# nyashiki/nshogi-engine

Hardware: AMD Instinct MI355X
Metric: NN evals/sec at batch=512 (higher is better)
Workload: dtype f16m6 (f16 main term + e2m3 MX correction terms with per-32-channel E8M0 scales, f32 accumulate)

## Files before the change

### nshogi-engine_amd/csrc/kernels/mfma_tile.h

```cpp
#ifndef NSG_MFMA_TILE_H
#define NSG_MFMA_TILE_H

#include "kernels.h"

#include <atomic>
#include <type_traits>

namespace nsg {
namespace tile {

typedef float f32x4 __attribute__((ext_vector_type(4)));
typedef unsigned int u32x4 __attribute__((ext_vector_type(4)));
typedef unsigned int u32x2 __attribute__((ext_vector_type(2)));
typedef __bf16 bf16x8 __attribute__((ext_vector_type(8)));
typedef _Float16 f16x8 __attribute__((ext_vector_type(8)));

enum Mode { kConv = 0, kHeads = 1, kDense = 2 };

#ifdef NSG_COOP_SC1_STORES
constexpr bool kCoopSameXcd = false;
#else
constexpr bool kCoopSameXcd = true;
#endif
#ifdef NSG_COOP_NO_KEEP
constexpr bool kCoopKeepOwnSlice = false;
#else
constexpr bool kCoopKeepOwnSlice = true;
#endif
#ifdef NSG_NO_EDGE_ROWS_ONE_BOARD
constexpr bool kEdgeRowsOneBoard = false;
#else
constexpr bool kEdgeRowsOneBoard = true;
#endif

template <int MODE, int SIZE, int NWAVES, int NBUF = 2>
struct Geom {
    static constexpr bool kBoards = (MODE == kConv);
    static constexpr int kRows = kBoards ? SIZE * 81 : SIZE * 16;
    static constexpr int kMF = (kRows + 15) / 16;
    static constexpr int kEntries = kBoards ? SIZE * 110 + 24 : kMF * 16;
    static constexpr int kPlane = (kEntries * 16 + 7 * 16 + 255) / 256 * 256;
    static constexpr int kPlaneStride = kPlane + 16;
    static_assert(7 * kPlaneStride + kEntries * 16 <= 8 * kPlane, "the eight skewed planes must fit the buffer");
    static constexpr int kBuf = 8 * kPlane;
    static constexpr int kLds = NBUF * kBuf;
    static constexpr int kEpi = kLds;
    static constexpr int kRowTabOff = (kEpi > kLds ? kEpi : kLds) + 1024;
    static constexpr int kLdsAlloc = kRowTabOff + 1024;
    static constexpr int kThreads = NWAVES * 64;
    static constexpr int kItems = (2 * kMF + NWAVES - 1) / NWAVES;
    static constexpr int kTaps = kBoards ? 9 : 1;
};

template <bool BOARDS>
__device__ __forceinline__ int entryOfRow(int m) {
    if constexpr (BOARDS) {
        const int b = m / 81;
        const int sq = m - b * 81;
        const int y = sq / 9;
        const int x = sq - y * 9;
        return 24 + b * 110 + (y + 1) * 10 + x;
    } else {
        return m;
    }
}

template <class G, bool SHIFT = false>
__device__ __forceinline__ void zeroHalo(unsigned char* smem, int tid) {
    static_assert(G::kBoards, "board images only");
    constexpr int kBoardsN = (G::kEntries - 24) / 110;
    constexpr int kHalo = 24 + 29 * kBoardsN;
    constexpr int kPlanes = G::kLds / G::kPlane;
    const int lane = tid & 63, wave = tid >> 6;
    constexpr int kWavesN = G::kThreads / 64;
#pragma unroll
    for (int h0 = 0; h0 < kHalo; h0 += 64) {
        const int h = h0 + lane;
        int e = h;
        if (h0 + 63 >= 24) {
            const int q = h - 24, b = q / 29, r = q - b * 29;
            const int within = r < 10 ? r : (r < 19 ? (r - 9) * 10 + 9 : 81 + r);
            e = h < 24 ? h : 24 + b * 110 + within;
        }
        e = h < kHalo ? e : 0;
#pragma unroll
        for (int pl = 0; pl < (kPlanes + kWavesN - 1) / kWavesN; ++pl) {
            int plane = pl * kWavesN + wave;
            plane = plane < kPlanes ? plane : kPlanes - 1;
            if constexpr (SHIFT) {
                unsigned char* z = smem + e * 16 + (plane >> 3) * G::kBuf + (plane & 7) * G::kPlaneStride + ((plane & 7) == 7 ? 8 : 0);
                *reinterpret_cast<u32x2*>(z) = u32x2{0u, 0u};
                *reinterpret_cast<u32x2*>(z + 8) = u32x2{0u, 0u};
            } else {
                *reinterpret_cast<u32x4*>(smem + e * 16 + (plane >> 3) * G::kBuf + (plane & 7) * G::kPlaneStride) = u32x4{0u, 0u, 0u, 0u};
            }
        }
    }
}

template <int PREC>
__device__ __forceinline__ void mfmaSlab(f32x4& acc, const u32x4& w, const u32x4& a) {
    if constexpr (PREC == kFp32) {
        acc = __builtin_amdgcn_mfma_f32_16x16x4f32(__uint_as_float(w.x), __uint_as_float(a.x), acc, 0, 0, 0);
        acc = __builtin_amdgcn_mfma_f32_16x16x4f32(__uint_as_float(w.y), __uint_as_float(a.y), acc, 0, 0, 0);
        acc = __builtin_amdgcn_mfma_f32_16x16x4f32(__uint_as_float(w.z), __uint_as_float(a.z), acc, 0, 0, 0);
        acc = __builtin_amdgcn_mfma_f32_16x16x4f32(__uint_as_float(w.w), __uint_as_float(a.w), acc, 0, 0, 0);
    } else if constexpr (PREC == kFp16 || PREC == kF16x3) {
        acc = __builtin_amdgcn_mfma_f32_16x16x32_f16(__builtin_bit_cast(f16x8, w), __builtin_bit_cast(f16x8, a), acc, 0, 0, 0);
    } else {
        acc = __builtin_amdgcn_mfma_f32_16x16x32_bf16(__builtin_bit_cast(bf16x8, w), __builtin_bit_cast(bf16x8, a), acc, 0, 0, 0);
    }
}

template <int PREC>
__device__ __forceinline__ uint16_t toBits16(float v) {
    if constexpr (PREC == kFp16 || PREC == kF16x3) {
        return __builtin_bit_cast(uint16_t, (_Float16)v);
    } else {
        return __builtin_bit_cast(uint16_t, (__bf16)v);
    }
}
template <int PREC>
__device__ __forceinline__ uint32_t packPair(float lo, float hi) {
    return (uint32_t)toBits16<PREC>(lo) | ((uint32_t)toBits16<PREC>(hi) << 16);
}
template <int PREC>
__device__ __forceinline__ float unpackLo(uint32_t v) {
    if constexpr (PREC == kFp16) {
        return (float)__builtin_bit_cast(_Float16, (uint16_t)(v & 0xffffu));
    } else {
        return __uint_as_float(v << 16);
    }
}
__device__ __forceinline__ void splitF16(float v, uint16_t& hi, uint16_t& lo) {
    v = fminf(fmaxf(v, -65000.f), 65000.f);
    const _Float16 h = (_Float16)v;
    const _Float16 l = (_Float16)(v - (float)h);
    hi = __builtin_bit_cast(uint16_t, h);
    lo = __builtin_bit_cast(uint16_t, l);
}
// ... 203 lines not shown
    }
    static constexpr Tab kTab = make();
    static constexpr int kN = kTab.n, kMain = kTab.nMain, kX = kTab.nX;
    static constexpr int slab(int u) { return kTab.slab[u]; }
    static constexpr int mainOrd(int u) { return kTab.mainOrd[u]; }
    static constexpr int xOrd(int u) { return kTab.xOrd[u]; }
    static constexpr int mainSlab(int o) { return kTab.mainSlab[o]; }
    static constexpr int xSlab(int j) { return kTab.xSlab[j]; }
    static constexpr bool kXCyclic = kX >= 2 && kX % 2 == 0;
    static_assert(kMain % 3 == 0, "three f16 weight sets must carry across chunk pairs");
    static_assert(kX == 0 || kTab.xOrd[0] < 0 || kXCyclic, "a pair must not start with an MX slab it requests at its top");
};

template <class OS, int MF, bool PERM, int WIN, class ER>
struct StepSeq {
    static constexpr int kMax = (27 * MF + WIN - 1) / WIN * WIN;
    struct Tab {
        int n, padded;
        short pos[kMax], frag[kMax], index[27 * MF], xord[kMax];
    };
    static constexpr bool active(int u, int f) { return !PERM || ER::needTap(f, OS::slab(u) / 3); }
    static constexpr Tab make() {
        Tab t{};
        int n = 0;
        for (int u = 0; u < OS::kN; ++u)
            for (int f = 0; f < MF; ++f) {
                t.index[u * MF + f] = (short)(active(u, f) ? n : -1);
                if (active(u, f)) {
                    t.pos[n] = (short)u;
                    t.frag[n] = (short)f;
                    ++n;
                }
            }
        t.n = n;
        t.padded = (n + WIN - 1) / WIN * WIN;
        for (int q = n; q < kMax; ++q) { t.pos[q] = 0; t.frag[q] = -1; }
        int nx = 0;
        for (int q = 0; q < kMax; ++q) {
            t.xord[q] = (short)nx;
            if (q < n && OS::slab(t.pos[q]) % 3 == 2) ++nx;
        }
        return t;
    }
    static constexpr Tab kTab = make();
    static constexpr int kReal = kTab.n;
    static constexpr int kSteps = kTab.padded;
    static constexpr int pos(int q) { return kTab.pos[q]; }
    static constexpr int frag(int q) { return kTab.frag[q]; }
    static constexpr int index(int u, int f) { return kTab.index[u * MF + f]; }
    static constexpr int xord(int q) { return kTab.xord[q]; }
};

template <int PREC, int MODE, int SIZE, int NFRAG, int NWAVES, int RES, int MS = 1, int KS = 1, int SS = 1, int PART = 0, bool COOP = false,
          bool KEEP = false>
__device__ __forceinline__ void tileBody(const Args& A, unsigned char* smem, bool zeroLds, bool haveOwn = false) {
    static_assert(!KEEP || (COOP && SIZE == 1 && MS == 1 && KS > 1 && PREC == kF16m6), "own slice kept in LDS: cooperative K-split tiles");
    static_assert(!COOP || (isMx(PREC) && MODE == kConv && NFRAG == 4), "cooperative trunk: MX conv tiles");
    static_assert(SS == 1 || (isMx(PREC) && MODE == kConv && SIZE == 2 && MS == 1 && KS == 1 && NWAVES % SS == 0 && PART < SS),
                  "slab split: two-board MX conv tiles");
    using G = Geom<MODE, SIZE, NWAVES, (isMx(PREC) ? (KS > 1 ? 8 : 4) : 2)>;
    static_assert(KS == 1 || (isMx(PREC) && MODE == kConv && SIZE == 1 && NWAVES % KS == 0),
                  "K split: kF16m8 one-board conv tiles");
    constexpr bool kRowWG = (MS > 1 && KS > 1);
    const bool hasRes = (RES == 1) || (RES == 2 && A.res != nullptr);
    NSG_STAMP_DECL
    NSG_STAMP(0);
    constexpr bool kM8 = isMx(PREC);
    constexpr bool kM6 = (PREC == kF16m6);
    constexpr int ES = (PREC == kFp32 || PREC == kF16x3 || kM8) ? 4 : 2;
    constexpr bool kSplit = (PREC == kF16x3);
    static_assert(!kM8 || (MODE == kConv && NFRAG == 4), "kF16m8: full trunk-conv tiles only");
    static_assert(NFRAG == 1 || NFRAG == 2 || NFRAG == 4, "fragments per wave");
    static_assert(MS == 1 || (MODE == kConv && SIZE == 1 && G::kMF % MS == 0 && (KS > 1 || NWAVES % MS == 0) &&
                              (NFRAG < 4 || isMx(PREC))),
                  "row split: one-board conv tiles (small tiles, or kF16m8 full-channel tiles)");
    constexpr int kMFw = G::kMF / MS;
#ifdef NSG_NO_EDGE_ROWS
    constexpr bool kPerm = false;
#else
    constexpr bool kPerm = isMx(PREC) && MODE == kConv && NFRAG == 4 && MS == 1 && KS == 1 && (SIZE == 2 || (SIZE == 1 && kEdgeRowsOneBoard));
#endif
    using EdgeRows = std::conditional_t<SIZE == 1, EdgeRows1, EdgeRowsT<SS == 1>>;
    static_assert(!kPerm || kMFw == EdgeRows::kMF, "edge-packed rows: one table row per fragment");

    int tidOpaque = threadIdx.x;
    asm volatile("" : "+v"(tidOpaque));
    const int tid = tidOpaque;
    const int lane = tid & 63;
    const int wave = __builtin_amdgcn_readfirstlane(tid >> 6);
    const int li = lane & 15;
    const int g = lane >> 4;
    const size_t row0 = (size_t)blockIdx.x * G::kRows;
    int nkc = A.kdim * ES / 128;
    int kc0 = 0;
    if constexpr (MODE == kDense) {
        const int per = nkc / A.kSplits;
        kc0 = blockIdx.z * per;
        nkc = per;
    }
    const int nft = A.cout / 16;
    const int waveGroup = (blockIdx.y * NWAVES + wave) / (kRowWG ? KS : MS * KS * SS);
    const int fBase = (MS > 1) ? (kRowWG ? (int)blockIdx.z : wave % MS) * kMFw : 0;
    const int rowLimit = kRowWG ? ((fBase + kMFw) * 16 < G::kRows ? (fBase + kMFw) * 16 : G::kRows) : G::kRows;
    const size_t lastRow = G::kBoards ? ~(size_t)0 : (size_t)(A.totalRows - 1);

    const int sli = lane >> 3, sg = lane & 7;
    size_t srcOff[G::kItems];
    int dstOff[G::kItems];
    bool itemOk[G::kItems];
// ... 12 lines not shown
    if constexpr (kTileBuf) {
        xrs = __builtin_amdgcn_make_buffer_rsrc(const_cast<unsigned char*>(A.x) + row0 * (size_t)A.kdim * ES, 0, 0x7fffffff, 0x00027000);
#pragma unroll
        for (int k = 0; k < G::kItems; ++k) srcRel[k] = (int)(srcOff[k] - row0 * (size_t)A.kdim * ES);
    }
    auto tileLoad = [&](int k, int chunk) -> u32x4 {
        if constexpr (kTileBuf) return __builtin_bit_cast(u32x4, __builtin_amdgcn_raw_buffer_load_b128(xrs, srcRel[k], chunk * 128, COOP ? 16  : 0));
        else return *reinterpret_cast<const u32x4*>(A.x + srcOff[k] + (size_t)chunk * 128);
    };
    u32x4 st[G::kItems];
#ifdef NSG_MX_SPLIT_READ
    constexpr bool kShiftLo = (PREC == kF16m6) && MODE == kConv;
#else
    constexpr bool kShiftLo = false;
#endif
    auto stageStore = [](unsigned char* p_, const u32x4& v_) {
        if constexpr (kShiftLo) {
            *reinterpret_cast<u32x2*>(p_) = u32x2{v_.x, v_.y};
            *reinterpret_cast<u32x2*>(p_ + 8) = u32x2{v_.z, v_.w};
        } else {
            *reinterpret_cast<u32x4*>(p_) = v_;
        }
    };
    constexpr bool kResident = isMx(PREC) && KS > 1;
    constexpr int kResChunks = 8;
    constexpr int kOwnChunks = KEEP ? 2 * (NWAVES / KS) : 0;
    [[maybe_unused]] const int ownChunk0 = (int)blockIdx.y * kOwnChunks;
    u32x4 stAll[kResident ? kResChunks : 1][G::kItems];
    if constexpr (kResident) {
#pragma unroll
        for (int c = 0; c < kResChunks; ++c) {
            if (KEEP && haveOwn && c >= ownChunk0 && c < ownChunk0 + kOwnChunks) continue;
#pragma unroll
            for (int k = 0; k < G::kItems; ++k)
                stAll[c][k] = __builtin_bit_cast(u32x4, __builtin_amdgcn_raw_buffer_load_b128(
                    xrs, c < nkc ? srcRel[k] : 0x7ffffff0, c * 128, COOP ? 16  : 0));
        }
        __builtin_amdgcn_sched_barrier(0);
        NSG_STAMP(4);
    }
#pragma unroll
    for (int k = 0; k < G::kItems; ++k) {
        const int wid = wave + k * NWAVES;
        const int c = sg;
        const int mm = itemOk[k] ? wid * 8 + sli : 0;
        const int okOff = c * G::kPlaneStride + entryOfRow<G::kBoards>(mm) * 16 + ((kShiftLo && c == 7) ? 8 : 0), okMask = -(int)itemOk[k];
        dstOff[k] = (okOff & okMask) | ((G::kLds + lane * 16) & ~okMask);
    }

    int abase[kMFw];
    constexpr int kTabParts = KS > 1 ? KS : SS;
    constexpr int kTabFrags = (kMFw + kTabParts - 1) / kTabParts * kTabParts;
    static_assert(!kPerm || (kTabFrags + 1) * 64 <= 1024, "epilogue row table");
#define NSG_COMPUTE_ABASE \
_Pragma("unroll") \
    for (int f = 0; f < kMFw; ++f) { \
        [[maybe_unused]] int eb = 0, ey = 0, ex = 0; \
        [[maybe_unused]] bool eok = true; \
        if constexpr (kPerm) eok = EdgeRows::square(f, li, eb, ey, ex); \
        const int m = kPerm ? (eok ? eb * 81 + ey * 9 + ex : -1) : (fBase + f) * 16 + li; \
        if constexpr (kPerm) { \
            static_assert(NFRAG * 16 * ES == 256, "edge-packed rows: 256-byte row slices (4 rows per instruction)"); \
            if (wave == 0 && g == 0) { \
                reinterpret_cast<unsigned*>(smem + G::kRowTabOff)[(f * 4 + (li & 3)) * 4 + (li >> 2)] = \
                    m >= 0 ? (unsigned)m * (unsigned)(A.cout * ES) : ~0u; \
                 \
                if (f == kMFw - 1) { \
                    _Pragma("unroll") for (int fx = kMFw; fx <= kTabFrags; ++fx) \
                        reinterpret_cast<unsigned*>(smem + G::kRowTabOff)[(fx * 4 + (li & 3)) * 4 + (li >> 2)] = ~0u; \
                } \
            } \
        } \
        if constexpr (G::kBoards) { \
            const int p = kPerm ? (eok ? 24 + eb * 110 + (ey + 1) * 10 + ex : 11) \
                                : ((m < G::kRows) ? entryOfRow<true>(m) : 11); \
            abase[f] = g * G::kPlaneStride + (p - 11) * 16; \
        } else { \
            abase[f] = g * G::kPlaneStride + m * 16; \
        } \
    }
    if constexpr (!kPerm) { NSG_COMPUTE_ABASE }

#define NSG_PIN_ACC_AGPR                                                                 \
    _Pragma("unroll") for (int f = 0; f < kMFw; ++f) {                                   \
        _Pragma("unroll") for (int j = 0; j < NFRAG; ++j) asm volatile("" : "+a"(acc[f][j])); \
    }
#define NSG_STAGE_LOAD(KC)                                                               \
    _Pragma("unroll") for (int k = 0; k < G::kItems; ++k) {                              \
        st[k] = *reinterpret_cast<const u32x4*>(A.x + srcOff[k] + (size_t)(KC) * 128);   \
    }
#define NSG_STAGE_WRITE(BUF)                                                             \
    _Pragma("unroll") for (int k = 0; k < G::kItems; ++k) {                              \
        stageStore(smem + (itemOk[k] ? (BUF) * G::kBuf : 0) + dstOff[k], st[k]);         \
    }

    f32x4 acc[kMFw][NFRAG];
#pragma unroll
    for (int f = 0; f < kMFw; ++f)
#pragma unroll
        for (int j = 0; j < NFRAG; ++j) acc[f][j] = f32x4{0.f, 0.f, 0.f, 0.f};

    if constexpr (kM8) {
        using Q = M8Seq<G::kTaps>;
        using OS = OwnSeq<SS, PART>;
        static_assert(G::kTaps == 9, "3x3 taps");
        constexpr int kWin = 9, kD = 7;
#ifdef NSG_NO_SPREAD_LOADS
        constexpr bool kSpread = false;
#else
        constexpr bool kSpread = kMFw > NFRAG;
#endif
        using ST = StepSeq<OS, kMFw, kPerm, kWin, EdgeRows>;
        constexpr int kReal = ST::kReal;
        constexpr int kSteps = ST::kSteps;
        constexpr int kPad = kSteps - kReal;
        static_assert(kSteps % kWin == 0 && kPad < kD, "window slot must carry across chunk pairs");
        constexpr int kOwn = OS::kN;
        constexpr int kLoadSlabs = kOwn >= 20 ? (G::kItems < 6 ? G::kItems : 6) : (kOwn >= 12 ? 3 : 1);
        constexpr int kLoadSlabA = kOwn >= 20 ? 2 : 0, kWriteA = kOwn >= 20 ? 12 : (kOwn >= 12 ? 6 : 3);
        constexpr int kLoadSlabB = kOwn >= 20 ? 13 : kWriteA, kWriteB = kOwn >= 20 ? 25 : (kOwn >= 12 ? 12 : kOwn - 1);
        static_assert(kLoadSlabA + kLoadSlabs <= kWriteA && kLoadSlabB + kLoadSlabs <= kWriteB && kWriteB < kOwn, "tile staging order");
        constexpr int kBarStep = kReal - kD;
        constexpr int kWriteStepA = ST::index(kWriteA, 0), kWriteStepB = ST::index(kWriteB, 0) < kBarStep ? ST::index(kWriteB, 0) : kBarStep - 1;
        static_assert(kWriteStepA >= 0 && ST::index(kWriteB, 0) >= 0 && kWriteStepA < kWriteStepB, "fragment 0 runs every tap");
        static_assert(kWriteStepB < kBarStep, "tile staging order");
        auto tapOff = [](int t) constexpr { return ((t / 3 - 1) * 10 + (t % 3 - 1) + 11) * 16; };
        const int offp8 = (g >> 1) * G::kBuf + (4 + 2 * (g & 1) - g) * G::kPlaneStride;
        constexpr bool kPackX = kM6;
        const int mainSet = nft * 1024, xSet = nft * (kPackX ? 1600 : 2048);
        const int tapStride = 2 * mainSet + xSet, pairStride = G::kTaps * tapStride;
        int tapS = tapStride, mainS = mainSet;
        auto mainOff = [&](int s) { return (s / 3) * tapS + (s % 3) * mainS; };
        auto xOff = [&](int s) { return (s / 3) * tapS + 2 * mainS; };
        constexpr bool kStage = (KS == 1);
        const int kpart = (KS > 1) ? wave % KS : 0;
        const int npairs = nkc / 2 / KS;
        const int pair0 = kpart * npairs;
        const __amdgpu_buffer_rsrc_t wrs = __builtin_amdgcn_make_buffer_rsrc(const_cast<u32x4*>(A.w), 0, 0x7fffffff, 0x00027000);
        int wc = pair0 * pairStride;
        const int wg4 = waveGroup * NFRAG * 1024;
        const int wg8 = kPackX ? waveGroup * 6400 : waveGroup * NFRAG * 2048;
        const int lane16 = lane * 16, lane8 = lane * 8, lane4 = lane * 4;
        auto ld16 = [&](int off_, int imm_) { return __builtin_bit_cast(u32x4, __builtin_amdgcn_raw_buffer_load_b128(wrs, lane16 + imm_, off_, 0)); };
        auto ld8 = [&](int off_, int imm_) { return __builtin_bit_cast(u32x2, __builtin_amdgcn_raw_buffer_load_b64(wrs, lane8 + imm_, off_, 0)); };
        auto ld4 = [&](int off_, int imm_) { return (uint32_t)__builtin_amdgcn_raw_buffer_load_b32(wrs, lane4 + imm_, off_, 0); };
        u32x4 w4[OS::kMain > 0 ? 3 : 1][NFRAG];
        u32x4 w8[OS::kX > 0 ? 2 : 1][NFRAG][kPackX ? 1 : 2];
        [[maybe_unused]] u32x2 w8b[OS::kX > 0 ? 2 : 1][NFRAG];
        [[maybe_unused]] uint32_t w8s[OS::kX > 0 ? 2 : 1];
#define NSG_M8_LOADX(SET_, OFF_, J_)                                                                            \
        _Pragma("unroll") for (int j_ = 0; j_ < NFRAG; ++j_) {                                                  \
            if ((J_) >= 0 && j_ != (J_)) continue;                                                              \
            if constexpr (kPackX) {                                                                             \
                w8[SET_][j_][0] = ld16(wc + (OFF_) + wg8, j_ * 1024);                                           \
                w8b[SET_][j_] = ld8(wc + (OFF_) + wg8 + 4096, j_ * 512);                                        \
                if ((J_) < 0 ? j_ == 0 : (J_) == 0) w8s[SET_] = ld4(wc + (OFF_) + wg8 + 4096, 2048);            \
            } else {                                                                                            \
                _Pragma("unroll") for (int h_ = 0; h_ < 2; ++h_)                                                \
                    w8[SET_][j_][kPackX ? 0 : h_] = ld16(wc + (OFF_) + wg8 + (j_ >> 1) * 4096, ((j_ & 1) * 2 + h_) * 1024); \
            }                                                                                                   \
        }
        if constexpr (OS::kMain > 0) {
#pragma unroll
            for (int o = 0; o < 2; ++o)
#pragma unroll
                for (int j = 0; j < NFRAG; ++j) w4[o][j] = ld16(wc + mainOff(OS::mainSlab(o)) + wg4, j * 1024);
        }
        if constexpr (OS::kXCyclic) { NSG_M8_LOADX(0, xOff(OS::xSlab(0)), -1) }

        if constexpr (kStage) {
        u32x4 st1[G::kItems];
#pragma unroll
        for (int k = 0; k < G::kItems; ++k) st[k] = tileLoad(k, 0);
#pragma unroll
        for (int k = 0; k < G::kItems; ++k) st1[k] = tileLoad(k, 1);
        NSG_STAMP(4);
        if constexpr (kPerm) { NSG_COMPUTE_ABASE }
        if (zeroLds) zeroHalo<G, kShiftLo>(smem, tid);
        __syncthreads();
        NSG_STAMP(5);
        NSG_STAGE_WRITE(0)
#pragma unroll
        for (int k = 0; k < G::kItems; ++k)
            stageStore(smem + (itemOk[k] ? G::kBuf : 0) + dstOff[k], st1[k]);
        __syncthreads();
        } else {
            constexpr int kChunks = kResChunks;
            if constexpr (kPerm) { NSG_COMPUTE_ABASE }
            if (zeroLds) zeroHalo<G, kShiftLo>(smem, tid);
            __syncthreads();
            NSG_STAMP(5);
#pragma unroll
            for (int c = 0; c < kChunks; ++c) {
                if (KEEP && haveOwn && c >= ownChunk0 && c < ownChunk0 + kOwnChunks) continue;
#pragma unroll
                for (int k = 0; k < G::kItems; ++k)
                    if (__builtin_expect(c < nkc, 1)) stageStore(smem + (itemOk[k] ? c * G::kBuf : 0) + dstOff[k], stAll[c][k]);
            }
            __syncthreads();
        }
        NSG_STAMP(1);

        constexpr bool kSplitRead = kShiftLo && OS::kX > 0;
        const int offB = offp8 + G::kPlaneStride + 8 * (g & 1);
        u32x4 aw[kWin][kSplitRead ? 1 : 2];
        [[maybe_unused]] u32x2 aw45[kSplitRead ? kWin : 1];
        [[maybe_unused]] uint32_t awS[kSplitRead ? kWin : 1];
#define NSG_M8_REQ(QQ, CUR, NXT)                                                                  \
        if (ST::frag((QQ) % kSteps) >= 0) {                                                       \
            const int q_ = (QQ) % kSteps;                                                         \
            const unsigned char* b_ = ((QQ) >= kSteps) ? (NXT) : (CUR);                           \
            const int s_ = OS::slab(ST::pos(q_)), f_ = ST::frag(q_);                              \
            if (Q::isX(s_)) {                                                                     \
                const unsigned char* ap_ = b_ + abase[f_] + offp8 + tapOff(Q::tap(s_));           \
                aw[(QQ) % kWin][0] = *reinterpret_cast<const u32x4*>(ap_);                        \
                [[maybe_unused]] const unsigned char* ap2_ = b_ + abase[f_] + offB + tapOff(Q::tap(s_)); \
                if constexpr (kSplitRead) {                                                       \
                    aw45[(QQ) % kWin] = *reinterpret_cast<const u32x2*>(ap2_);                    \
                    awS[(QQ) % kWin] = *reinterpret_cast<const uint32_t*>(ap2_ + 12);             \
                } else if constexpr (kShiftLo) {                                                  \
                    aw[(QQ) % kWin][kSplitRead ? 0 : 1] = *reinterpret_cast<const u32x4*>(ap2_);  \
                } else {                                                                          \
                    aw[(QQ) % kWin][kSplitRead ? 0 : 1] = *reinterpret_cast<const u32x4*>(ap_ + G::kPlaneStride); \
                }                                                                                 \
            } else {                                                                              \
                aw[(QQ) % kWin][0] = *reinterpret_cast<const u32x4*>(                             \
                    b_ + Q::half(s_) * G::kBuf + abase[f_] + tapOff(Q::tap(s_)));                 \
            }                                                                                     \
        }
        const unsigned char* first = kStage ? smem : smem + (size_t)(2 * pair0) * G::kBuf;
#pragma unroll
        for (int q = 0; q < kD - kPad; ++q) NSG_M8_REQ(q, first, first)

        for (int kp = 0; kp < npairs; ++kp) {
            const unsigned char* abuf = kStage ? smem + ((2 * kp) & 3) * G::kBuf : smem + (size_t)(2 * (pair0 + kp)) * G::kBuf;
            const unsigned char* nbuf = kStage ? smem + ((2 * kp + 2) & 3) * G::kBuf
                                               : (kp + 1 < npairs ? abuf + 2 * G::kBuf : abuf);
            [[maybe_unused]] const int nextA = (kp + 1 < npairs) ? 2 * kp + 2 : 2 * kp;
// ... 387 lines not shown
                            const f32x4 rr = *reinterpret_cast<const f32x4*>(A.res + e + j * 16);
#pragma unroll
                            for (int i = 0; i < 4; ++i) v[j * 4 + i] += rr[i];
                        } else {
                            const u32x2 rr = *reinterpret_cast<const u32x2*>(A.res + e + j * 8);
                            v[j * 4 + 0] += unpackLo<PREC>(rr.x); v[j * 4 + 1] += unpackHi<PREC>(rr.x);
                            v[j * 4 + 2] += unpackLo<PREC>(rr.y); v[j * 4 + 3] += unpackHi<PREC>(rr.y);
                        }
                    }
                }
                if (A.relu) {
#pragma unroll
                    for (int i = 0; i < NFRAG * 4; ++i) v[i] = reluF(v[i]);
                }
#pragma unroll
                for (int j = 0; j < NFRAG; ++j) {
                    if constexpr (PREC == kFp32) {
                        *reinterpret_cast<f32x4*>(A.y + e + j * 16) = f32x4{v[j * 4], v[j * 4 + 1], v[j * 4 + 2], v[j * 4 + 3]};
                    } else {
                        *reinterpret_cast<u32x2*>(A.y + e + j * 8) =
                            u32x2{packPair<PREC>(v[j * 4], v[j * 4 + 1]), packPair<PREC>(v[j * 4 + 2], v[j * 4 + 3])};
                    }
                }
            }
        }
        NSG_STAMP(3);
        return;
    }

#ifdef NSG_EXP_RUNTIME
    if constexpr (MODE == kConv && NFRAG == 4 && isMx(PREC)) {
        if (A.exp & 2) {
#pragma unroll
            for (int f = 0; f < kMFw; ++f)
#pragma unroll
                for (int j = 0; j < NFRAG; ++j) asm volatile("" ::"v"(acc[f][j]));
            NSG_STAMP(3);
            return;
        }
    }
#endif
    if constexpr (MODE == kConv && NFRAG == 4) {
        constexpr int kParts = KS > 1 ? KS : SS;
        constexpr int kMFe = (kMFw + kParts - 1) / kParts;
        const int fBaseE = fBase + ((KS > 1) ? (wave % KS) * kMFe : PART * kMFe);
        constexpr int kRowB = NFRAG * 16 * ES;
        constexpr int kRowS = kRowB + 16;
        constexpr int kNP = kRowB / 64;
        constexpr int kPPR = kRowB / 16;
        constexpr int kRPI = 64 / kPPR;
        constexpr int kIPF = 16 / kRPI;
        constexpr int kFragBytes = 16 * kRowS;
        constexpr int kEpiWave = G::kEpi / NWAVES / 16 * 16;
        constexpr int kRegions = (kEpiWave / kFragBytes) < 1 ? 1 : ((kEpiWave / kFragBytes) > 4 ? 4 : (kEpiWave / kFragBytes));
        static_assert(kFragBytes <= kEpiWave, "epilogue staging does not fit");
        unsigned char* ebuf = smem + wave * kEpiWave;
        const size_t rowBytes = (size_t)A.cout * ES;
        const size_t sliceOff = (size_t)waveGroup * kRowB;
        auto pieceOff = [&](int k) -> int {
            if constexpr (kSplit || kM6) return (g >> 1) * 128 + (g & 1) * 32 + (k & 1) * 16 + (k >> 1) * 64;
            else if constexpr (kM8)
                return (g >> 1) * 128 + (k < 2 ? (g & 1) * 32 + k * 16 : 64 + (k - 2) * 32 + (g & 1) * 16);
            else return g * (kRowB / 4) + k * 16;
        };
        const bool outX3 = kM8 && A.outF16x3;
        auto pieceOffX3 = [&](int k) -> int { return (g >> 1) * 128 + (g & 1) * 32 + (k & 1) * 16 + (k >> 1) * 64; };
        const int lrow = lane / kPPR;
        const int lpc = lane % kPPR;
        const unsigned laneOff = (unsigned)lrow * (unsigned)rowBytes + (unsigned)lpc * 16u;
        const size_t tileOff = (row0 + (kPerm ? (size_t)0 : (size_t)fBaseE * 16)) * rowBytes + sliceOff;
        const unsigned char* resBase = A.res + tileOff;
        unsigned char* yBase = A.y + tileOff;
        [[maybe_unused]] __amdgpu_buffer_rsrc_t resRs, yRs;
        if constexpr (COOP) {
            resRs = __builtin_amdgcn_make_buffer_rsrc(const_cast<unsigned char*>(resBase), 0, 0x7fffffff, 0x00027000);
            yRs = __builtin_amdgcn_make_buffer_rsrc(yBase, 0, 0x7fffffff, 0x00027000);
        }
        auto resLoad = [&](size_t off_) -> u32x4 {
            if constexpr (COOP) return __builtin_bit_cast(u32x4, __builtin_amdgcn_raw_buffer_load_b128(resRs, (int)off_, 0, 16));
            else return *reinterpret_cast<const u32x4*>(resBase + off_);
        };
        auto outStore = [&](size_t off_, const u32x4& v_) {
            if constexpr (COOP) __builtin_amdgcn_raw_buffer_store_b128(v_, yRs, (int)off_, 0, kCoopSameXcd ? 0 : 16);
            else *reinterpret_cast<u32x4*>(yBase + off_) = v_;
        };
        [[maybe_unused]] const unsigned permLane = (unsigned)lpc * 16u;
        const int fBasePerm = (KS > 1) ? (wave % KS) * kMFe : PART * kMFe;
        auto rowOffs = [&](int f) -> u32x4 {
            if constexpr (kPerm) return *reinterpret_cast<const u32x4*>(smem + G::kRowTabOff + ((fBasePerm + f) * 4 + lrow) * 16);
            else return u32x4{0u, 0u, 0u, 0u};
        };
        auto rowOk = [&](int f, int it, const u32x4& ro) -> bool {
            if constexpr (kPerm) return (SIZE == 2 && KS == 1 && PART * kMFe + f < EdgeRows::kMF - 1) || ro[it] != ~0u;
            else return (fBaseE + f) * 16 + it * kRPI + lrow < rowLimit;
        };
        auto rowByte = [&](int f, int it, const u32x4& ro) -> size_t {
            if constexpr (kPerm) return (size_t)(ro[it] + permLane);
            else return (size_t)(f * 16 + it * kRPI) * rowBytes + laneOff;
        };

        constexpr int kPreFrags = (RES != 1 || minWavesPerSimd<MODE, SIZE, NWAVES, NFRAG, PREC>() > 1)
                                      ? 0 : (kMFe * kIPF <= 32 ? kMFe : 32 / kIPF);
        u32x4 rpre[kPreFrags ? kPreFrags : 1][kIPF];
        if constexpr (kPreFrags > 0) {
#pragma unroll
            for (int f = 0; f < kPreFrags; ++f) {
                const u32x4 ro = rowOffs(f);
#pragma unroll
                for (int it = 0; it < kIPF; ++it) {
                    rpre[f][it] = u32x4{0u, 0u, 0u, 0u};
                    if (__builtin_expect(rowOk(f, it, ro), 1))
                        rpre[f][it] = resLoad(rowByte(f, it, ro));
                }
            }
        }

        static_assert(kRegions >= 2, "the pipelined epilogue needs two staging regions per wave");
        [[maybe_unused]] int entLi[KEEP ? kMFe : 1], entLL[KEEP ? kMFe : 1][kIPF];
        if constexpr (KEEP) {
            static_assert(kRowB == 256 && kIPF == 4, "image staging: 256-byte row slices");
            const int slice_ = waveGroup * 2 * G::kBuf;
            auto entryByte = [&](int m_) { return m_ < G::kRows ? slice_ + (34 + m_ + ((m_ * 57) >> 9)) * 16 : -1; };
            auto rowOfFrag = [&](int fg_, int r_) -> int {
                if constexpr (kPerm) {
                    int b_ = 0, y_ = 0, x_ = 0;
                    const bool ok_ = EdgeRows::square(fg_ < EdgeRows::kMF ? fg_ : 0, r_, b_, y_, x_) && fg_ < EdgeRows::kMF;
                    return ok_ ? y_ * 9 + x_ : G::kRows;
                } else {
                    return fg_ * 16 + r_;
                }
            };
#pragma unroll
            for (int f = 0; f < kMFe; ++f) {
                entLi[f] = entryByte(rowOfFrag(fBaseE + f, li));
#pragma unroll
                for (int it = 0; it < kIPF; ++it) entLL[f][it] = entryByte(rowOfFrag(fBaseE + f, it * kRPI + lrow));
            }
        }
        auto stageAt = [&](int f, int rowIsLi, int it, int piece_) -> unsigned char* {
            if constexpr (KEEP) {
                const int e_ = rowIsLi ? entLi[f] : entLL[f][it];
                return smem + (e_ < 0 ? G::kLds + lane * 16 : e_ + (piece_ >> 3) * G::kBuf + (piece_ & 7) * G::kPlaneStride);
            } else {
                return ebuf + (f % kRegions) * kFragBytes + (rowIsLi ? li : it * kRPI + lrow) * kRowS + piece_ * 16;
            }
        };
        u32x4 rpp[2][kNP];
        u32x4 tt[kIPF];
#pragma unroll
        for (int i = -1; i <= kMFe; ++i) {
            [[maybe_unused]] u32x4 roS = u32x4{0u, 0u, 0u, 0u}, roR = u32x4{0u, 0u, 0u, 0u};
            if (i >= 1) {
                const int f = i - 1;
#pragma unroll
                for (int it = 0; it < kIPF; ++it)
                    tt[it] = *reinterpret_cast<const u32x4*>(stageAt(f, 0, it, lpc));
                roS = rowOffs(f);
            }
            if (hasRes && i + 1 < kMFe) {
                const int f = i + 1;
                if (f >= kPreFrags) roR = rowOffs(f);
                const u32x4 ro = roR;
#pragma unroll
                for (int it = 0; it < kIPF; ++it) {
                    u32x4 t = u32x4{0u, 0u, 0u, 0u};
                    if (f < kPreFrags) {
                        t = rpre[f < kPreFrags ? f : 0][it];
                    } else {
                        if (__builtin_expect(rowOk(f, it, ro), 1))
                            t = resLoad(rowByte(f, it, ro));
                    }
                    *reinterpret_cast<u32x4*>(stageAt(f, 0, it, lpc)) = t;
                }
#pragma unroll
                for (int k = 0; k < kNP; ++k) {
                    const int po = (kM6 && k >= 2) ? (g >> 1) * 128 + 96 + (k - 2) * 16 : pieceOff(k);
                    rpp[f & 1][k] = *reinterpret_cast<const u32x4*>(stageAt(f, 1, 0, po / 16));
                }
            }
            if (i >= 0 && i < kMFe) {
                const int f = i;
                float v[NFRAG * 4];
#pragma unroll
                for (int j = 0; j < NFRAG; ++j)
#pragma unroll
                    for (int r = 0; r < 4; ++r) v[j * 4 + r] = fmaf(acc[f][j][r], A.accScale, bv[j * 4 + r]);
                [[maybe_unused]] unsigned char* lrowp = ebuf + (f % kRegions) * kFragBytes + li * kRowS;
                if (hasRes) {
                    const u32x4* rp = rpp[f & 1];
                    if constexpr (PREC == kFp32) {
#pragma unroll
                        for (int k = 0; k < 4; ++k)
#pragma unroll
                            for (int i = 0; i < 4; ++i) v[k * 4 + i] += __uint_as_float(rp[k][i]);
                    } else if constexpr (kSplit) {
#pragma unroll
                        for (int k = 0; k < 2; ++k)
#pragma unroll
                            for (int i = 0; i < 4; ++i) {
// ... 110 lines not shown
                            sb[d] = sw.y;
                        }
                        const uint32_t mbits = __builtin_bit_cast(uint32_t, __builtin_convertvector(f32x2{mh, ml}, f16x2));
                        const uint32_t mhb = mbits & 0xffffu, mlb = mbits >> 16;
                        op[0] = u32x4{hpv[0], hpv[1], hpv[2], hpv[3]};
                        op[1] = u32x4{hpv[4], hpv[5], hpv[6], hpv[7]};
                        const u32x16 src = {sa[0], sa[1], sa[2], sa[3], sa[4], sa[5], sa[6], sa[7],
                                            sb[0], sb[1], sb[2], sb[3], sb[4], sb[5], sb[6], sb[7]};
                        const u32x2v mm = __builtin_amdgcn_permlane16_swap(mhb, mlb, false, false);
                        const uint32_t e5 = (mm.x > mm.y ? mm.x : mm.y) >> 10;
                        const uint32_t e8 = e5 + 110u;
                        u32x6 blk;
                        const float sc = __uint_as_float(e8 << 23);
                        asm("v_cvt_scalef32_pk32_fp6_f16 %0, %1, %2" : "=&v"(blk) : "v"(src), "v"(sc));
                        op[2] = u32x4{blk.s0, blk.s1, blk.s2, blk.s3};
                        op[3] = u32x4{blk.s4, blk.s5, e8, e8};
                    } else {
                        typedef float f32x2 __attribute__((ext_vector_type(2)));
                        typedef _Float16 f16x2 __attribute__((ext_vector_type(2)));
#pragma unroll
                        for (int d = 0; d < 4; ++d) {
                            f32x2 hf[2], lf[2];
#pragma unroll
                            for (int q = 0; q < 2; ++q) {
                                const int c = 4 * d + 2 * q;
                                const f32x2 x = {__builtin_amdgcn_fmed3f(v[c], floorV, 65000.f),
                                                 __builtin_amdgcn_fmed3f(v[c + 1], floorV, 65000.f)};
                                const f16x2 h = __builtin_convertvector(x, f16x2);
                                op[c >> 3][(c & 7) >> 1] = __builtin_bit_cast(uint32_t, h);
                                const f32x2 hx = __builtin_convertvector(h, f32x2);
                                const f32x2 lx = (x - hx) * (float)(1 << kM8LoShift);
                                hf[q] = f32x2{__builtin_amdgcn_fmed3f(hx[0], -448.f, 448.f), __builtin_amdgcn_fmed3f(hx[1], -448.f, 448.f)};
                                lf[q] = f32x2{__builtin_amdgcn_fmed3f(lx[0], -448.f, 448.f), __builtin_amdgcn_fmed3f(lx[1], -448.f, 448.f)};
                            }
                            int h8 = __builtin_amdgcn_cvt_pk_fp8_f32(hf[0][0], hf[0][1], 0, false);
                            h8 = __builtin_amdgcn_cvt_pk_fp8_f32(hf[1][0], hf[1][1], h8, true);
                            int l8 = __builtin_amdgcn_cvt_pk_fp8_f32(lf[0][0], lf[0][1], 0, false);
                            l8 = __builtin_amdgcn_cvt_pk_fp8_f32(lf[1][0], lf[1][1], l8, true);
                            op[2][d] = (uint32_t)h8;
                            op[3][d] = (uint32_t)l8;
                        }
                    }
                } else {
#pragma unroll
                    for (int k = 0; k < 2; ++k)
#pragma unroll
                        for (int i = 0; i < 4; ++i) op[k][i] = packPair<PREC>(v[k * 8 + 2 * i], v[k * 8 + 2 * i + 1]);
                }
#pragma unroll
                for (int k = 0; k < kNP; ++k) {
                    if constexpr (KEEP) *reinterpret_cast<u32x4*>(stageAt(f, 1, 0, (__builtin_expect(outX3, false) ? pieceOffX3(k) : pieceOff(k)) / 16)) = op[k];
                    else *reinterpret_cast<u32x4*>(lrowp + (__builtin_expect(outX3, false) ? pieceOffX3(k) : pieceOff(k))) = op[k];
                }
            }
            if (i >= 1) {
                const int f = i - 1;
                const u32x4 ro = roS;
#pragma unroll
                for (int it = 0; it < kIPF; ++it) {
#ifdef NSG_EXP_RUNTIME
                    asm volatile("" ::"v"(tt[it]));
                    if (__builtin_expect(rowOk(f, it, ro) && !(A.exp & 1), 1))
#else
                    if (__builtin_expect(rowOk(f, it, ro), 1))
#endif
                        outStore(rowByte(f, it, ro), tt[it]);
                }
            }
        }
#ifdef NSG_DIAG_STAMPS
        asm volatile("s_waitcnt vmcnt(0)" ::: "memory");
#endif
        NSG_STAMP(3);
        return;
    }

#pragma unroll
    for (int f = 0; f < G::kMF; ++f) {
        const int m = f * 16 + li;
        const size_t grow = row0 + m;
        const bool rowOk = G::kBoards ? (m < G::kRows) : (grow <= lastRow);
        if (!rowOk) continue;
        float v[NFRAG * 4];
#pragma unroll
        for (int j = 0; j < NFRAG; ++j)
#pragma unroll
            for (int r = 0; r < 4; ++r) v[j * 4 + r] = fmaf(acc[f][j][r], A.accScale, bv[j * 4 + r]);

        if constexpr (MODE == kHeads) {
            const int b = (int)(grow / 81);
            const int sq = (int)(grow - (size_t)b * 81);
            const int vc = A.valueChannels;
#pragma unroll
            for (int i = 0; i < NFRAG * 4; ++i) {
                const int n = cbase + i;
                if (n < vc) {
                    const float r = reluF(v[i]);
                    const size_t e = (size_t)b * A.vfeatStride + (size_t)sq * vc + n;
                    if constexpr (kSplit) {
                        const int kk = sq * vc + n;
                        uint16_t hb, lb;
                        splitF16(r, hb, lb);
                        unsigned char* row = A.vfeat + (size_t)b * A.vfeatStride * 4 + (size_t)(kk >> 5) * 128 + (kk & 31) * 2;
                        *reinterpret_cast<uint16_t*>(row) = hb;
                        *reinterpret_cast<uint16_t*>(row + 64) = lb;
                    } else if constexpr (PREC == kFp32) {
                        reinterpret_cast<float*>(A.vfeat)[e] = r;
                    } else {
                        reinterpret_cast<uint16_t*>(A.vfeat)[e] = toBits16<PREC>(r);
                    }
                } else if (n < vc + 27) {
                    A.policy[(size_t)b * 2187 + (size_t)(n - vc) * 81 + sq] = v[i];
                }
            }
        } else {
            float* out = reinterpret_cast<float*>(A.y) + (size_t)blockIdx.z * A.partStride + grow * (size_t)A.cout + cbase;
#pragma unroll
            for (int j = 0; j < NFRAG; ++j)
                *reinterpret_cast<f32x4*>(out + j * 4) =
                    f32x4{acc[f][j][0] * A.accScale, acc[f][j][1] * A.accScale, acc[f][j][2] * A.accScale, acc[f][j][3] * A.accScale};
        }
    }
}

template <int PREC, int MODE, int SIZE, int NFRAG, int NWAVES, bool HAS_RES, int MS = 1, int KS = 1, int SS = 1>
__global__ __launch_bounds__(NWAVES * 64, (minWavesPerSimd<MODE, SIZE, NWAVES, NFRAG, PREC>())) void tileKernel(
    const unsigned char* x, const u32x4* w, const unsigned char* res, unsigned char* y, const float* bias,
    int kdim, int cout, int flags , float accScale, const ArgsTail T) {
    extern __shared__ __attribute__((aligned(16))) unsigned char smem[];
    const Args A{x, w, bias, res, y, T.policy, T.vfeat, kdim, cout, T.totalRows, flags & 1, T.valueChannels,
                 T.vfeatStride, accScale, (flags >> 1) & 1, T.kSplits, T.partStride, T.stamps, flags >> 2};
    if constexpr (SS == 1) {
        tileBody<PREC, MODE, SIZE, NFRAG, NWAVES, HAS_RES ? 1 : 0, MS, KS>(A, smem, true);
    } else {
        const int part = __builtin_amdgcn_readfirstlane((int)(threadIdx.x >> 6)) % SS;
        if (part == 0) tileBody<PREC, MODE, SIZE, NFRAG, NWAVES, HAS_RES ? 1 : 0, MS, KS, SS, 0>(A, smem, true);
        else if (part == 1) tileBody<PREC, MODE, SIZE, NFRAG, NWAVES, HAS_RES ? 1 : 0, MS, KS, SS, 1>(A, smem, true);
        else if constexpr (SS > 2) {
            if (part == 2) tileBody<PREC, MODE, SIZE, NFRAG, NWAVES, HAS_RES ? 1 : 0, MS, KS, SS, 2>(A, smem, true);
            else tileBody<PREC, MODE, SIZE, NFRAG, NWAVES, HAS_RES ? 1 : 0, MS, KS, SS, 3>(A, smem, true);
        }
    }
}

template <int PREC, int SIZE, int NFRAG, int NWAVES>
__global__ __launch_bounds__(NWAVES * 64, (minWavesPerSimd<kConv, SIZE, NWAVES, NFRAG, PREC>())) void trunkKernel(
    const Args* __restrict__ layers, int nLayers, int skewTicks) {
    extern __shared__ __attribute__((aligned(16))) unsigned char smem[];
    if (skewTicks > 0) {
        const unsigned long long t0 = __builtin_amdgcn_s_memrealtime();
        const unsigned long long wait = (unsigned long long)skewTicks * ((blockIdx.x >> 3) & 7);
        while (__builtin_amdgcn_s_memrealtime() - t0 < wait) __builtin_amdgcn_s_sleep(16);
    }
    for (int l = 0; l < nLayers; ++l) {
        const Args A = layers[l];
        if (A.res) tileBody<PREC, kConv, SIZE, NFRAG, NWAVES, 1>(A, smem, true);
        else tileBody<PREC, kConv, SIZE, NFRAG, NWAVES, 0>(A, smem, true);
        __syncthreads();
    }
}

template <int PREC, int NFRAG, int NWAVES, int MS, int KS>
__global__ __launch_bounds__(NWAVES * 64, 1) void coopTrunkKernel(const Args* __restrict__ layers, int nLayers, int boards,
                                                                  unsigned* flags, unsigned flagBase, int* status, int faultBoard) {
    extern __shared__ __attribute__((aligned(16))) unsigned char smem[];
    using G = Geom<kConv, 1, NWAVES, 8>;
    if ((int)blockIdx.x >= boards) return;
    const int members = (int)(gridDim.y * gridDim.z), me = (int)(blockIdx.z * gridDim.y + blockIdx.y);
    if ((int)blockIdx.x == faultBoard && me == 1) return;
    unsigned xcc = 0;
    if constexpr (kCoopSameXcd) {
        asm volatile("s_getreg_b32 %0, hwreg(HW_REG_XCC_ID, 0, 4)" : "=s"(xcc));
        if (faultBoard == -2 && me == 1) xcc ^= 1u;
    }
    int* gaveUp = reinterpret_cast<int*>(smem + G::kLdsAlloc);
    unsigned* mine = flags + (size_t)blockIdx.x * members;
    if (threadIdx.x == 0) *gaveUp = 0;
    for (int l = 0; l < nLayers; ++l) {
        const Args A = layers[l];
        asm volatile("" ::"s"(A.x), "s"(A.w), "s"(A.res), "s"(A.y), "s"(A.bias), "s"(A.kdim), "s"(A.cout), "s"(A.relu), "s"(A.accScale),
                     "s"(A.outF16x3));
        if (l > 0) {
            if ((int)threadIdx.x < members && (int)threadIdx.x != me) {
                int spins = 0;
                unsigned seen;
                while (((seen = __hip_atomic_load(mine + threadIdx.x, __ATOMIC_RELAXED, __HIP_MEMORY_SCOPE_AGENT)) & 0xffffffu) < flagBase + (unsigned)l) {
                    if ((++spins & 255) == 0 &&
                        (spins > (1 << 21) || __hip_atomic_load(status, __ATOMIC_RELAXED, __HIP_MEMORY_SCOPE_SYSTEM) != 0)) {
                        __hip_atomic_store(status, 1, __ATOMIC_RELAXED, __HIP_MEMORY_SCOPE_SYSTEM);
                        *gaveUp = 1;
                        seen = xcc << 24;
                        break;
                    }
                    __builtin_amdgcn_s_sleep(4);
                }
                if (kCoopSameXcd && (seen >> 24) != xcc) {
                    __hip_atomic_store(status, 2, __ATOMIC_RELAXED, __HIP_MEMORY_SCOPE_SYSTEM);
                    *gaveUp = 1;
                }
            }
            __syncthreads();
            if (*gaveUp) return;
        }
        constexpr bool kKeep = kCoopKeepOwnSlice && MS == 1;
        if (A.res) tileBody<PREC, kConv, 1, NFRAG, NWAVES, 1, MS, KS, 1, 0, true, kKeep>(A, smem, true, l > 0);
        else tileBody<PREC, kConv, 1, NFRAG, NWAVES, 0, MS, KS, 1, 0, true, kKeep>(A, smem, true, l > 0);
        asm volatile("s_waitcnt vmcnt(0)" ::: "memory");
        __syncthreads();
        if (threadIdx.x == 0) __hip_atomic_store(mine + me, (flagBase + (unsigned)(l + 1)) | (xcc << 24), __ATOMIC_RELAXED, __HIP_MEMORY_SCOPE_AGENT);
    }
// ... 143 lines not shown
```

Before: 204,500.

## Keep first input chunk pair in LDS across layers of persistent trunk kernel

In the persistent two-board f16m6 trunk kernel, wave 0 of the y==0 block writes its epilogue output for the first chunk pair straight into the LDS staging planes that the next layer reads. On later layers the tile then skips the global loads and stage writes for chunks 0-1 and only zeroes the halo of the remaining planes. The epilogue staging is moved into chunk buffers 2-3 and a small entry table is added. The aim is to cut global reads and a barrier-separated staging pass per layer, at the cost of extra LDS stores in the epilogue, fewer prefetched residual fragments, and correctness that depends on each block keeping the same boards and channel slice across layers.

```diff
diff --git a/nshogi-engine_amd/csrc/kernels/mfma_tile.h b/nshogi-engine_amd/csrc/kernels/mfma_tile.h
--- a/nshogi-engine_amd/csrc/kernels/mfma_tile.h
+++ b/nshogi-engine_amd/csrc/kernels/mfma_tile.h
@@ -26,6 +26,11 @@
 constexpr bool kCoopKeepOwnSlice = false;
 #else
 constexpr bool kCoopKeepOwnSlice = true;
+#endif
+#if defined(NSG_TRUNK_NO_KEEP0) || defined(NSG_MX_SPLIT_READ)
+constexpr bool kTrunkKeepPair0 = false;
+#else
+constexpr bool kTrunkKeepPair0 = true;
 #endif
 #ifdef NSG_NO_EDGE_ROWS_ONE_BOARD
 constexpr bool kEdgeRowsOneBoard = false;
@@ -65,12 +70,13 @@
     }
 }
 
-template <class G, bool SHIFT = false>
+template <class G, bool SHIFT = false, int P0 = 0>
 __device__ __forceinline__ void zeroHalo(unsigned char* smem, int tid) {
     static_assert(G::kBoards, "board images only");
     constexpr int kBoardsN = (G::kEntries - 24) / 110;
     constexpr int kHalo = 24 + 29 * kBoardsN;
     constexpr int kPlanes = G::kLds / G::kPlane;
+    static_assert(P0 >= 0 && P0 < kPlanes, "first plane");
     const int lane = tid & 63, wave = tid >> 6;
     constexpr int kWavesN = G::kThreads / 64;
 #pragma unroll
@@ -84,8 +90,8 @@
         }
         e = h < kHalo ? e : 0;
 #pragma unroll
-        for (int pl = 0; pl < (kPlanes + kWavesN - 1) / kWavesN; ++pl) {
-            int plane = pl * kWavesN + wave;
+        for (int pl = 0; pl < (kPlanes - P0 + kWavesN - 1) / kWavesN; ++pl) {
+            int plane = P0 + pl * kWavesN + wave;
             plane = plane < kPlanes ? plane : kPlanes - 1;
             if constexpr (SHIFT) {
                 unsigned char* z = smem + e * 16 + (plane >> 3) * G::kBuf + (plane & 7) * G::kPlaneStride + ((plane & 7) == 7 ? 8 : 0);
@@ -395,9 +401,11 @@
 };
 
 template <int PREC, int MODE, int SIZE, int NFRAG, int NWAVES, int RES, int MS = 1, int KS = 1, int SS = 1, int PART = 0, bool COOP = false,
-          bool KEEP = false>
-__device__ __forceinline__ void tileBody(const Args& A, unsigned char* smem, bool zeroLds, bool haveOwn = false) {
+          bool KEEP = false, bool OWN0 = false>
+__device__ __forceinline__ void tileBody(const Args& A, unsigned char* smem, bool zeroLds, bool haveOwn = false, bool keepNext = false) {
     static_assert(!KEEP || (COOP && SIZE == 1 && MS == 1 && KS > 1 && PREC == kF16m6), "own slice kept in LDS: cooperative K-split tiles");
+    static_assert(!OWN0 || (!COOP && !KEEP && PREC == kF16m6 && MODE == kConv && SIZE == 2 && NFRAG == 4 && MS == 1 && KS == 1 && SS == 1),
+                  "first chunk pair kept in LDS: the persistent two-board tile");
     static_assert(!COOP || (isMx(PREC) && MODE == kConv && NFRAG == 4), "cooperative trunk: MX conv tiles");
     static_assert(SS == 1 || (isMx(PREC) && MODE == kConv && SIZE == 2 && MS == 1 && KS == 1 && NWAVES % SS == 0 && PART < SS),
                   "slab split: two-board MX conv tiles");
@@ -516,6 +524,8 @@
     constexpr int kTabParts = KS > 1 ? KS : SS;
     constexpr int kTabFrags = (kMFw + kTabParts - 1) / kTabParts * kTabParts;
     static_assert(!kPerm || (kTabFrags + 1) * 64 <= 1024, "epilogue row table");
+    constexpr int kKeepTabOff = G::kRowTabOff + (kTabFrags + 1) * 64;
+    static_assert(!OWN0 || ((kTabFrags + 1) * 64 + kMFw * 16 <= 1024 && G::kEntries < 256), "kept-pair entry table");
 #define NSG_COMPUTE_ABASE \
 _Pragma("unroll") \
     for (int f = 0; f < kMFw; ++f) { \
@@ -539,6 +549,9 @@
             const int p = kPerm ? (eok ? 24 + eb * 110 + (ey + 1) * 10 + ex : 11) \
                                 : ((m < G::kRows) ? entryOfRow<true>(m) : 11); \
             abase[f] = g * G::kPlaneStride + (p - 11) * 16; \
+            if constexpr (OWN0) { \
+                if (wave == 0 && g == 0) smem[kKeepTabOff + f * 16 + li] = (unsigned char)(p == 11 ? 0 : p); \
+            } \
         } else { \
             abase[f] = g * G::kPlaneStride + m * 16; \
         } \
@@ -634,20 +647,28 @@
 
         if constexpr (kStage) {
         u32x4 st1[G::kItems];
-#pragma unroll
-        for (int k = 0; k < G::kItems; ++k) st[k] = tileLoad(k, 0);
-#pragma unroll
-        for (int k = 0; k < G::kItems; ++k) st1[k] = tileLoad(k, 1);
+        const bool own0 = OWN0 && haveOwn;
+        if (!own0) {
+#pragma unroll
+            for (int k = 0; k < G::kItems; ++k) st[k] = tileLoad(k, 0);
+#pragma unroll
+            for (int k = 0; k < G::kItems; ++k) st1[k] = tileLoad(k, 1);
+        }
         NSG_STAMP(4);
         if constexpr (kPerm) { NSG_COMPUTE_ABASE }
-        if (zeroLds) zeroHalo<G, kShiftLo>(smem, tid);
-        __syncthreads();
-        NSG_STAMP(5);
-        NSG_STAGE_WRITE(0)
-#pragma unroll
-        for (int k = 0; k < G::kItems; ++k)
-            stageStore(smem + (itemOk[k] ? G::kBuf : 0) + dstOff[k], st1[k]);
-        __syncthreads();
+        if (own0) {
+            if constexpr (OWN0) zeroHalo<G, kShiftLo, 16>(smem, tid);
+            NSG_STAMP(5);
+        } else {
+            if (zeroLds) zeroHalo<G, kShiftLo>(smem, tid);
+            __syncthreads();
+            NSG_STAMP(5);
+            NSG_STAGE_WRITE(0)
+#pragma unroll
+            for (int k = 0; k < G::kItems; ++k)
+                stageStore(smem + (itemOk[k] ? G::kBuf : 0) + dstOff[k], st1[k]);
+            __syncthreads();
+        }
         } else {
             constexpr int kChunks = kResChunks;
             if constexpr (kPerm) { NSG_COMPUTE_ABASE }
@@ -1141,9 +1162,10 @@
         constexpr int kIPF = 16 / kRPI;
         constexpr int kFragBytes = 16 * kRowS;
         constexpr int kEpiWave = G::kEpi / NWAVES / 16 * 16;
-        constexpr int kRegions = (kEpiWave / kFragBytes) < 1 ? 1 : ((kEpiWave / kFragBytes) > 4 ? 4 : (kEpiWave / kFragBytes));
+        constexpr int kRegions = OWN0 ? 3 : ((kEpiWave / kFragBytes) < 1 ? 1 : ((kEpiWave / kFragBytes) > 4 ? 4 : (kEpiWave / kFragBytes)));
         static_assert(kFragBytes <= kEpiWave, "epilogue staging does not fit");
-        unsigned char* ebuf = smem + wave * kEpiWave;
+        static_assert(!OWN0 || NWAVES * kRegions * kFragBytes <= 2 * G::kBuf, "epilogue staging of every wave inside chunk buffers 2-3");
+        unsigned char* ebuf = OWN0 ? smem + 2 * G::kBuf + wave * (kRegions * kFragBytes) : smem + wave * kEpiWave;
         const size_t rowBytes = (size_t)A.cout * ES;
         const size_t sliceOff = (size_t)waveGroup * kRowB;
         auto pieceOff = [&](int k) -> int {
@@ -1189,7 +1211,7 @@
         };
 
         constexpr int kPreFrags = (RES != 1 || minWavesPerSimd<MODE, SIZE, NWAVES, NFRAG, PREC>() > 1)
-                                      ? 0 : (kMFe * kIPF <= 32 ? kMFe : 32 / kIPF);
+                                      ? 0 : (kMFe * kIPF <= 32 ? kMFe : 32 / kIPF - (OWN0 ? 1 : 0));
         u32x4 rpre[kPreFrags ? kPreFrags : 1][kIPF];
         if constexpr (kPreFrags > 0) {
 #pragma unroll
@@ -1234,6 +1256,8 @@
                 return ebuf + (f % kRegions) * kFragBytes + (rowIsLi ? li : it * kRPI + lrow) * kRowS + piece_ * 16;
             }
         };
+        [[maybe_unused]] const bool keepOwn = OWN0 && keepNext && wave == 0 && blockIdx.y == 0;
+        [[maybe_unused]] const int keepLane = (g >> 1) * G::kBuf + (g & 1) * 2 * G::kPlaneStride;
         u32x4 rpp[2][kNP];
         u32x4 tt[kIPF];
 #pragma unroll
@@ -1450,6 +1474,17 @@
                     if constexpr (KEEP) *reinterpret_cast<u32x4*>(stageAt(f, 1, 0, (__builtin_expect(outX3, false) ? pieceOffX3(k) : pieceOff(k)) / 16)) = op[k];
                     else *reinterpret_cast<u32x4*>(lrowp + (__builtin_expect(outX3, false) ? pieceOffX3(k) : pieceOff(k))) = op[k];
                 }
+                if constexpr (OWN0) {
+                    static_assert(!OWN0 || (kM6 && kRowB == 256 && kNP == 4 && kMFe == kMFw), "kept pair: 256-byte row slices in the kF16m6 layout");
+                    if (keepOwn) {
+                        const int ent = smem[kKeepTabOff + f * 16 + li];
+#pragma unroll
+                        for (int k = 0; k < kNP; ++k) {
+                            const int kept = keepLane + ent * 16 + ((k & 1) + (k >> 1) * 4) * G::kPlaneStride;
+                            *reinterpret_cast<u32x4*>(smem + (ent == 0 ? G::kLds + lane * 16 : kept)) = op[k];
+                        }
+                    }
+                }
             }
             if (i >= 1) {
                 const int f = i - 1;
@@ -1552,8 +1587,9 @@
     }
     for (int l = 0; l < nLayers; ++l) {
         const Args A = layers[l];
-        if (A.res) tileBody<PREC, kConv, SIZE, NFRAG, NWAVES, 1>(A, smem, true);
-        else tileBody<PREC, kConv, SIZE, NFRAG, NWAVES, 0>(A, smem, true);
+        constexpr bool kOwn0 = kTrunkKeepPair0 && PREC == kF16m6 && SIZE == 2 && NFRAG == 4 && NWAVES == 4;
+        if (A.res) tileBody<PREC, kConv, SIZE, NFRAG, NWAVES, 1, 1, 1, 1, 0, false, false, kOwn0>(A, smem, true, l > 0, l + 1 < nLayers);
+        else tileBody<PREC, kConv, SIZE, NFRAG, NWAVES, 0, 1, 1, 1, 0, false, false, kOwn0>(A, smem, true, l > 0, l + 1 < nLayers);
         __syncthreads();
     }
 }
```

Result: slower. 198,400 (-3.0%).
